# jackroos/VL-BERT

Hardware: AMD Instinct MI355X
Metric: samples/sec VL-BERT-base pretrain (seq 64+36 regions) at 1/2/4/8 MI355X (higher is better)
Workload: dtype bf16; 1 GPU; VL-BERT-base 12-layer pretrain step (fwd+bwd+clip+AdamW), 64 text + 36 regions, precomputed 2048-d region features, dropout on; global_batch=256, per_gpu_batch=256, per_gpu_caption_samples=256, per_gpu_text_only_samples=0, module=ResNetVLBERTForPretraining, seq_len=101, parallelism=dp1, hipgraph=False, arch=gfx950:sramecc+:xnack-, cus=256, forced_exchange=False, ranks=1

## Files before the change

vl-bert_amd/csrc/embed.hip:

```cpp
#include "vlb_common.h"

#define EMB_MAX_IT 8

enum { KIND_PAD = 0, KIND_TEXT = 1, KIND_OBJ = 2, KIND_END = 3 };

__global__ void seq_layout_kernel(const uint8_t* __restrict__ text_mask, const uint8_t* __restrict__ obj_mask, int B, int T, int R,
                                  int S, int32_t* __restrict__ code, int32_t* __restrict__ text_len, int32_t* __restrict__ nobj,
                                  int32_t* __restrict__ text_rows, int32_t* __restrict__ obj_rows, float* __restrict__ attn_mask) {
  const int b = blockIdx.x;
  if (threadIdx.x != 0) return;
  int n = 0;
  for (int t = 0; t < T; ++t)
    if (text_mask[b * T + t]) code[b * S + n++] = (KIND_TEXT << 16) | t;
  const int tl = n;
  for (int r = 0; r < R; ++r) {
    if (obj_mask[b * R + r]) {
      obj_rows[b * R + r] = b * S + n;
      code[b * S + n++] = (KIND_OBJ << 16) | r;
    } else {
      obj_rows[b * R + r] = -1;
    }
  }
  const int no = n - tl;
  code[b * S + n++] = (KIND_END << 16);
  for (int s = n; s < S; ++s) code[b * S + s] = (KIND_PAD << 16);
  for (int s = 0; s < S; ++s) attn_mask[b * S + s] = (s < n) ? 1.f : 0.f;
  for (int t = 0; t < T; ++t) text_rows[b * T + t] = b * S + t;
  text_len[b] = tl;
  nobj[b] = no;
}

__global__ __launch_bounds__(256) void obj_prep_fwd_kernel(const float* __restrict__ boxes, long ldbox, const float* __restrict__ im_info, long ldinfo,
                                                           const int64_t* __restrict__ mvrc_ops, const float* __restrict__ mask_emb,
                                                           bf16_t* __restrict__ out, int B, int R, uint32_t drop_thr, float drop_scale,
                                                           const uint32_t* __restrict__ seedp, uint32_t tag) {
  const int row = blockIdx.x;
  const int b = row / R;
  const float* bx = boxes + (long)row * ldbox;
  bf16_t* o = out + (long)row * 4096;
  const int tid = threadIdx.x;
  const uint32_t seed = (drop_thr && seedp) ? *seedp : 0u;
  if (!(bx[0] > -1.5f)) {
    *(uint4*)(o + tid * 8) = make_uint4(0, 0, 0, 0);
    *(uint4*)(o + 2048 + tid * 8) = make_uint4(0, 0, 0, 0);
    return;
  }
  const float W = im_info[b * ldinfo + 0], Hh = im_info[b * ldinfo + 1];
  const float x1 = bx[0], y1 = bx[1], x2 = bx[2], y2 = bx[3];
  float pos[4];
  pos[0] = (x1 + x2) / 2 / W * 100;
  pos[1] = (y1 + y2) / 2 / Hh * 100;
  pos[2] = (x2 - x1) / W * 100;
  pos[3] = (y2 - y1) / Hh * 100;
  const bool masked = mvrc_ops && mvrc_ops[row] == 1;
  const float* feat = masked ? mask_emb : (bx + 4);
#pragma unroll
  for (int part = 0; part < 2; ++part) {
    const int e0 = part * 1024 + tid * 4;
    float cv[4], fv[4];
    {
      const int which = e0 >> 9, j0 = e0 & 511;
      const bool is_cos = j0 >= 256;
#pragma unroll
      for (int k = 0; k < 4; ++k) {
        const float dim = powf(1000.0f, (float)((j0 & 255) + k) / 256.0f);
        const float a = pos[which] / dim;
        cv[k] = is_cos ? cosf(a) : sinf(a);
      }
      const float4 f = *(const float4*)(feat + e0);
      fv[0] = f.x; fv[1] = f.y; fv[2] = f.z; fv[3] = f.w;
    }
    if (drop_thr) {
      const uint32_t ic = (uint32_t)row * 4096u + (uint32_t)e0, ifeat = ic + 2048u;
      const uint32_t h0 = vlb_rng_pair(seed, tag, ic >> 1), h1 = vlb_rng_pair(seed, tag, (ic >> 1) + 1);
      const uint32_t g0 = vlb_rng_pair(seed, tag, ifeat >> 1), g1 = vlb_rng_pair(seed, tag, (ifeat >> 1) + 1);
      cv[0] = ((h0 & 0xffffu) >= drop_thr) ? cv[0] * drop_scale : 0.f;
      cv[1] = ((h0 >> 16) >= drop_thr) ? cv[1] * drop_scale : 0.f;
      cv[2] = ((h1 & 0xffffu) >= drop_thr) ? cv[2] * drop_scale : 0.f;
      cv[3] = ((h1 >> 16) >= drop_thr) ? cv[3] * drop_scale : 0.f;
      fv[0] = ((g0 & 0xffffu) >= drop_thr) ? fv[0] * drop_scale : 0.f;
      fv[1] = ((g0 >> 16) >= drop_thr) ? fv[1] * drop_scale : 0.f;
      fv[2] = ((g1 & 0xffffu) >= drop_thr) ? fv[2] * drop_scale : 0.f;
      fv[3] = ((g1 >> 16) >= drop_thr) ? fv[3] * drop_scale : 0.f;
    }
    *(uint2*)(o + e0) = make_uint2(pack2bf(cv[0], cv[1]), pack2bf(cv[2], cv[3]));
    *(uint2*)(o + 2048 + e0) = make_uint2(pack2bf(fv[0], fv[1]), pack2bf(fv[2], fv[3]));
  }
}

__global__ __launch_bounds__(256) void zero_padded_rows_kernel(bf16_t* __restrict__ x, long ld, const float* __restrict__ boxes, long ldbox,
                                                               int rows, int H) {
  const int row = blockIdx.x * 4 + (threadIdx.x >> 6), lane = threadIdx.x & 63;
  if (row >= rows || boxes[(long)row * ldbox] > -1.5f) return;
  for (int c = lane * 8; c < H; c += 512) *(uint4*)(x + (long)row * ld + c) = make_uint4(0, 0, 0, 0);
}

extern "C" int vlb_zero_padded_rows_bf16(void* x, long ld, const float* boxes, long ldbox, int rows, int H, hipStream_t stream) {
  if (rows <= 0) return VLB_OK;
  VLB_CHECK_ARG(x && boxes && H > 0 && (H % 8) == 0 && (ld % 8) == 0, "vlb_zero_padded_rows_bf16: bad argument");
  hipLaunchKernelGGL(zero_padded_rows_kernel, dim3(vlb_cdiv(rows, 4)), dim3(256), 0, stream, (bf16_t*)x, ld, boxes, ldbox, rows, H);
  VLB_CHECK_LAUNCH("vlb_zero_padded_rows_bf16");
  return VLB_OK;
}

__global__ __launch_bounds__(256) void masked_colsum_kernel(const bf16_t* __restrict__ src, long lds, const int64_t* __restrict__ sel,
                                                            int rows, int C, float* __restrict__ dst, uint32_t drop_thr,
                                                            float drop_scale, const uint32_t* __restrict__ seedp, uint32_t tag,
                                                            uint32_t row_elems, uint32_t col_off) {
  const int c = blockIdx.x * 256 + threadIdx.x;
  if (c >= C) return;
  const uint32_t seed = (drop_thr && seedp) ? *seedp : 0u;
  float s = 0.f;
  for (int r = blockIdx.y; r < rows; r += gridDim.y) {
    if (sel[r] != 1) continue;
    float v = bf2f(src[(long)r * lds + c]);
    if (drop_thr) v = vlb_keep(seed, tag, (uint32_t)r * row_elems + col_off + (uint32_t)c, drop_thr) ? v * drop_scale : 0.f;
    s += v;
  }
  atomicAdd(dst + c, s);
}

struct EmbedParams {
  const int32_t* code;
  const int32_t* text_len;
  const int64_t* text_ids;
  const int64_t* text_type;
  const bf16_t* word_emb;
  const bf16_t* pos_emb;
  const bf16_t* type_emb;
  const bf16_t* end_emb;
  const bf16_t* text_vis; long tv_sb, tv_st;
  const bf16_t* obj_vis; long ov_sb, ov_sr;
  const bf16_t* obj_ling; long ol_sb, ol_sr;
  const int64_t* obj_ling_idx;
  const float* gamma; const float* beta;
  bf16_t* pre;
  float* stats;
  bf16_t* out;
  int B, T, R, S, H, V, P;
  float eps;
  uint32_t drop_thr; float drop_scale; const uint32_t* seed; uint32_t tag;
};
// ... 391 lines not shown
  VLB_CHECK_LAUNCH("vlb_seq_layout");
  return VLB_OK;
}

extern "C" int vlb_obj_prep_fwd(const float* boxes, long ldbox, const float* im_info, long ldinfo, const int64_t* mvrc_ops,
                                const float* mask_emb, void* out, int B, int R, float drop_p, const uint32_t* seed, uint32_t tag,
                                hipStream_t stream) {
  if (B * R <= 0) return VLB_OK;
  VLB_CHECK_ARG(ldbox >= 4 + 2048 && (ldbox % 4) == 0, "vlb_obj_prep_fwd: ldbox=%ld must be >= 2052 and a multiple of 4", ldbox);
  VLB_CHECK_ARG(boxes && im_info && out && ldinfo >= 2, "vlb_obj_prep_fwd: null argument or im_info rows narrower than (width, height): ldinfo=%ld",
                ldinfo);
  VLB_CHECK_ARG(!(drop_p > 0.f) || seed, "vlb_obj_prep_fwd: dropout needs a device seed pointer");
  const uint32_t thr = vlb_drop_thr(drop_p);
  hipLaunchKernelGGL(obj_prep_fwd_kernel, dim3(B * R), dim3(256), 0, stream, boxes, ldbox, im_info, ldinfo, mvrc_ops, mask_emb, (bf16_t*)out,
                     B, R, thr, vlb_drop_scale(thr), seed, tag);
  VLB_CHECK_LAUNCH("vlb_obj_prep_fwd");
  return VLB_OK;
}

extern "C" int vlb_masked_colsum(const void* src, long lds_, const int64_t* sel, int rows, int C, float* dst, float drop_p,
                                 const uint32_t* seed, uint32_t tag, uint32_t row_elems, uint32_t col_off, hipStream_t stream) {
  if (rows <= 0 || C <= 0) return VLB_OK;
  const uint32_t thr = vlb_drop_thr(drop_p);
  int gy = rows < 64 ? rows : 64;
  hipLaunchKernelGGL(masked_colsum_kernel, dim3(vlb_cdiv(C, 256), gy), dim3(256), 0, stream, (const bf16_t*)src, lds_, sel, rows, C,
                     dst, thr, vlb_drop_scale(thr), seed, tag, row_elems, col_off);
  VLB_CHECK_LAUNCH("vlb_masked_colsum");
  return VLB_OK;
}

extern "C" int vlb_embed_fwd(const int32_t* code, const int32_t* text_len, const int64_t* text_ids, const int64_t* text_type,
                             const void* word_emb, const void* pos_emb, const void* type_emb, const void* end_emb,
                             const void* text_vis, long tv_sb, long tv_st, const void* obj_vis, long ov_sb, long ov_sr,
                             const void* obj_ling, long ol_sb, long ol_sr, const int64_t* obj_ling_idx, const float* gamma,
                             const float* beta, void* pre, float* stats, void* out, int B, int T, int R, int S, int H, int V,
                             int P, float eps, float drop_p, const uint32_t* seed, uint32_t tag, hipStream_t stream) {
  VLB_CHECK_ARG(H > 0 && (H % 4) == 0 && H <= 256 * EMB_MAX_IT, "vlb_embed_fwd: unsupported H=%d", H);
  VLB_CHECK_ARG(code && text_len && text_ids && word_emb && pos_emb && type_emb && end_emb && text_vis && obj_vis && obj_ling,
                "vlb_embed_fwd: null input");
  VLB_CHECK_ARG(!(drop_p > 0.f) || seed, "vlb_embed_fwd: dropout needs a device seed pointer");
  EmbedParams p;
  p.code = code; p.text_len = text_len; p.text_ids = text_ids; p.text_type = text_type;
  p.word_emb = (const bf16_t*)word_emb; p.pos_emb = (const bf16_t*)pos_emb; p.type_emb = (const bf16_t*)type_emb;
  p.end_emb = (const bf16_t*)end_emb;
  p.text_vis = (const bf16_t*)text_vis; p.tv_sb = tv_sb; p.tv_st = tv_st;
  p.obj_vis = (const bf16_t*)obj_vis; p.ov_sb = ov_sb; p.ov_sr = ov_sr;
  p.obj_ling = (const bf16_t*)obj_ling; p.ol_sb = ol_sb; p.ol_sr = ol_sr; p.obj_ling_idx = obj_ling_idx;
  p.gamma = gamma; p.beta = beta; p.pre = (bf16_t*)pre; p.stats = stats; p.out = (bf16_t*)out;
  p.B = B; p.T = T; p.R = R; p.S = S; p.H = H; p.V = V; p.P = P; p.eps = eps;
// ... 109 lines not shown
```

vl-bert_amd/csrc/layernorm.hip:

```cpp
#include <stdlib.h>

#include "options.h"
#include "vlb_common.h"

#define LN_MAX_IT 8
#define LN_MAX_BLOCKS 1024

__device__ unsigned int g_vlb_ln_nonfinite = 0u;

template <int NIT>
struct Row4 {
  float v[NIT][4];
};

template <int NIT>
struct Raw4 {
  uint2 w[NIT];
};

template <int NIT>
__device__ __forceinline__ void raw_load_row(const bf16_t* x, int H, int lane, Raw4<NIT>& q) {
#pragma unroll
  for (int i = 0; i < NIT; ++i) q.w[i] = *(const uint2*)(x + min((lane + 64 * i) * 4, H - 4));
}
// ... 382 lines not shown
  for (int i = 0; i < NIT; ++i)
#pragma unroll
    for (int k = 0; k < 4; ++k) {
      mine[(i * 4 + k) * 64 + lane] = gsum[i][k];
      mine[LW + (i * 4 + k) * 64 + lane] = bsum[i][k];
    }
  __syncthreads();
  for (int q = threadIdx.x; q < 2 * LW; q += 256) {
    const float v = (red[q] + red[2 * LW + q]) + (red[4 * LW + q] + red[6 * LW + q]);
    if (ws) ws[(long)blockIdx.x * 2 * LW + q] = v;
    else red[q] = v;
  }
  if (ws) return;
  __syncthreads();
  for (int c = threadIdx.x; c < 2 * H; c += 256) {
    const int which = c >= H, col = c - which * H, chunk = col >> 2;
    const float v = red[which * LW + (((chunk >> 6) * 4 + (col & 3)) << 6) + (chunk & 63)];
    float* dst = which ? dbeta : dgamma;
    if (dst) atomicAdd(dst + col, v);
  }
}


__global__ __launch_bounds__(256) void ln_param_finalize_kernel(const float* __restrict__ ws, int nslab, int LW, float* __restrict__ dgamma,
                                                                float* __restrict__ dbeta, int H, int cpl_log2) {
  __shared__ float part[4][64];
  const int tx = threadIdx.x & 63, ty = threadIdx.x >> 6;
  const int q = blockIdx.x * 64 + tx;
  float s = 0.f;
  for (int r = blockIdx.y * 4 + ty; r < nslab; r += 4 * gridDim.y) s += ws[(long)r * 2 * LW + q];
  part[ty][tx] = s;
  __syncthreads();
  if (ty == 0) {
    s = (part[0][tx] + part[1][tx]) + (part[2][tx] + part[3][tx]);
    const int r = q % LW, cpl = 1 << cpl_log2;
    const int col = ((r & 63) + 64 * (r >> (6 + cpl_log2))) * cpl + ((r >> 6) & (cpl - 1));
    if (col < H) {
      if (q < LW) { if (dgamma) atomicAdd(dgamma + col, s); }
      else if (dbeta) atomicAdd(dbeta + col, s);
    }
  }
}


extern "C" int vlb_layernorm_fwd(const void* x, long ldx, const float* gamma, const float* beta, void* y, long ldy,
                                 float* stats, int rows, int H, float eps, int x_f16, hipStream_t stream) {
  if (rows <= 0) return VLB_OK;
  VLB_CHECK_ARG(H > 0 && (H % 4) == 0 && H <= 256 * LN_MAX_IT, "vlb_layernorm_fwd: unsupported H=%d", H);
  VLB_CHECK_ARG((ldx % 4) == 0 && (ldy % 4) == 0, "vlb_layernorm_fwd: row strides must be multiples of 4");
  const int rpw_opt = vlb_opt(VLB_OPT_LN_FWD_ROWS);
  const int rpw = (rpw_opt == 1 || rpw_opt == 2 || rpw_opt == 4) ? rpw_opt : (rows >= 2 * 256 * 32 ? 2 : 1);
#define LN_FWD_R(NIT, RPW)                                                                                                              \
  hipLaunchKernelGGL((layernorm_fwd_kernel<NIT, RPW>), dim3(vlb_cdiv(rows, 4 * RPW)), dim3(256), 0, stream, (const bf16_t*)x, ldx, gamma, \
// ... 111 lines not shown
                     workspace, rows, H, x_f16, false, stream);
}

extern "C" int vlb_layernorm_bwd_slabs(int rows) {
  if (rows <= 0) return 0;
  const int blocks = ln_bwd_blocks(rows);
  return blocks > 32 ? blocks : 0;
}

struct LnFinalizeBatch {
  const float* ws[32];
  float* dgamma[32];
  float* dbeta[32];
  int nslab[32];
};

__global__ __launch_bounds__(256) void ln_param_finalize_batch_kernel(const LnFinalizeBatch b, int LW, int H, int cpl_log2) {
  __shared__ float part[4][64];
  const int e = blockIdx.z;
  const float* ws = b.ws[e];
  const int nslab = b.nslab[e];
  const int tx = threadIdx.x & 63, ty = threadIdx.x >> 6;
  const int q = blockIdx.x * 64 + tx;
  float s = 0.f;
  for (int r = blockIdx.y * 4 + ty; r < nslab; r += 4 * gridDim.y) s += ws[(long)r * 2 * LW + q];
  part[ty][tx] = s;
  __syncthreads();
  if (ty == 0) {
    s = (part[0][tx] + part[1][tx]) + (part[2][tx] + part[3][tx]);
    const int r = q % LW, cpl = 1 << cpl_log2;
    const int col = ((r & 63) + 64 * (r >> (6 + cpl_log2))) * cpl + ((r >> 6) & (cpl - 1));
    if (col < H) {
      if (q < LW) { if (b.dgamma[e]) atomicAdd(b.dgamma[e] + col, s); }
      else if (b.dbeta[e]) atomicAdd(b.dbeta[e] + col, s);
    }
  }
}

extern "C" int vlb_ln_param_finalize_batch(int n, const float* const* ws, const int* nslab, float* const* dgamma, float* const* dbeta,
                                           int H, hipStream_t stream) {
  if (n <= 0) return VLB_OK;
  VLB_CHECK_ARG(n <= 32 && ws && nslab && dgamma && dbeta, "vlb_ln_param_finalize_batch: 1..32 entries");
  VLB_CHECK_ARG(H > 0 && (H % 8) == 0 && H <= 2048, "vlb_ln_param_finalize_batch: unsupported H=%d", H);
  LnFinalizeBatch b;
  for (int i = 0; i < n; ++i) {
    VLB_CHECK_ARG(ws[i] && nslab[i] > 0, "vlb_ln_param_finalize_batch: entry %d has no partial vectors", i);
    b.ws[i] = ws[i]; b.nslab[i] = nslab[i]; b.dgamma[i] = dgamma[i]; b.dbeta[i] = dbeta[i];
  }
// ... 14 lines not shown
```

vl-bert_amd/csrc/loss.hip:

```cpp
#include "vlb_common.h"

__device__ __forceinline__ void online_merge(float& m, float& s, float m2, float s2) {
  const float mn = fmaxf(m, m2);
  if (mn == -INFINITY) return;
  s = s * __expf(m - mn) + s2 * __expf(m2 - mn);
  m = mn;
}

__device__ __forceinline__ void block_online_reduce(float& m, float& s, float* sh) {
#pragma unroll
  for (int o = 32; o > 0; o >>= 1) {
    const float m2 = __shfl_xor(m, o, 64), s2 = __shfl_xor(s, o, 64);
    online_merge(m, s, m2, s2);
  }
  const int wave = threadIdx.x >> 6, lane = threadIdx.x & 63;
  __syncthreads();
  if (lane == 0) {
    sh[wave * 2] = m;
    sh[wave * 2 + 1] = s;
  }
  __syncthreads();
  m = sh[0];
  s = sh[1];
#pragma unroll
// ... 54 lines not shown
  block_online_reduce(m, s, sh);
  const float lse = m + __logf(s);
  const float nv = fmaxf(*n_valid, 1.f);
  if (threadIdx.x == 0) atomicAdd(loss_out, (lse - bf2f(x[label])) / nv);
  const float sc = gscale / nv;
  __syncthreads();
  for (int c = threadIdx.x * 8; c < ldv; c += 2048) {
    const uint4 w = *(const uint4*)(x + c);
    const uint32_t ww[4] = {w.x, w.y, w.z, w.w};
    uint32_t o[4];
#pragma unroll
    for (int k = 0; k < 4; ++k) {
      const int c0 = c + 2 * k, c1 = c0 + 1;
      float g0 = (c0 < V) ? __expf(bflo(ww[k]) - lse) : 0.f;
      float g1 = (c1 < V) ? __expf(bfhi(ww[k]) - lse) : 0.f;
      if (c0 == label) g0 -= 1.f;
      if (c1 == label) g1 -= 1.f;
      o[k] = pack2bf(g0 * sc, g1 * sc);
    }
    *(uint4*)(x + c) = make_uint4(o[0], o[1], o[2], o[3]);
  }
}

__global__ __launch_bounds__(1024) void mlm_compact_kernel(const int64_t* __restrict__ labels, const int32_t* __restrict__ src_rows, int n,
                                                           int n_split, int V, int cap, int32_t* __restrict__ sel_pos,
                                                           int32_t* __restrict__ sel_src, int64_t* __restrict__ labels_c,
                                                           float* __restrict__ count0, float* __restrict__ count1,
                                                           int32_t* __restrict__ overflow) {
  __shared__ int wsum[16];
  __shared__ int total_s, n0_s;
  const int tid = threadIdx.x, lane = tid & 63, wave = tid >> 6;
  const int per = (n + 1023) / 1024, lo = tid * per, hi = min(n, lo + per);
  int c = 0, c0 = 0;
  for (int i = lo; i < hi; ++i) {
    const bool lab = labels[i] >= 0 && labels[i] < V;
    c += lab;
    c0 += lab && i < n_split;
  }
  int incl = c;
#pragma unroll
  for (int o = 1; o < 64; o <<= 1) {
    const int t = __shfl_up(incl, o, 64);
    if (lane >= o) incl += t;
  }
  if (lane == 63) wsum[wave] = incl;
  const float f0 = wave_sum((float)c0);
  __syncthreads();
  if (tid == 0) {
    int run = 0;
    for (int w = 0; w < 16; ++w) { const int t = wsum[w]; wsum[w] = run; run += t; }
    total_s = run;
    n0_s = 0;
  }
  __syncthreads();
  if (lane == 0 && f0 != 0.f) atomicAdd(&n0_s, (int)f0);
  __syncthreads();
  int k = wsum[wave] + incl - c;
  for (int i = lo; i < hi; ++i) {
    const long lb = labels[i];
    if (lb >= 0 && lb < V) {
      if (k < cap) {
        sel_pos[k] = i;
        sel_src[k] = src_rows[i];
        labels_c[k] = lb;
      }
      ++k;
    }
  }
  const int total = total_s;
  for (int q = total + tid; q < cap; q += 1024) {
    sel_pos[q] = -1;
    sel_src[q] = -1;
    labels_c[q] = -1;
  }
  if (tid == 0) {
    const int kept = min(total, cap), n0 = min(n0_s, kept);
    *count0 = (float)n0;
    *count1 = (float)(kept - n0);
    if (total > cap) *overflow = 1;
  }
}

extern "C" int vlb_mlm_compact(const int64_t* labels, const int32_t* src_rows, int n, int n_split, int V, int cap, int32_t* sel_pos,
                               int32_t* sel_src, int64_t* labels_c, float* count0, float* count1, int32_t* overflow, hipStream_t stream) {
  VLB_CHECK_ARG(labels && src_rows && sel_pos && sel_src && labels_c && count0 && count1 && overflow, "vlb_mlm_compact: null argument");
  VLB_CHECK_ARG(n > 0 && cap > 0 && n_split >= 0 && n_split <= n, "vlb_mlm_compact: bad sizes");
  hipLaunchKernelGGL(mlm_compact_kernel, dim3(1), dim3(1024), 0, stream, labels, src_rows, n, n_split, V, cap, sel_pos, sel_src, labels_c,
                     count0, count1, overflow);
  VLB_CHECK_LAUNCH("vlb_mlm_compact");
  return VLB_OK;
}

extern "C" int vlb_ce_fwd_bwd_compact(void* logits, long ld, int rows, int V, const int64_t* labels_c, const float* count0,
                                      const float* count1, float gscale, float* loss_out0, float* loss_out1, hipStream_t stream) {
  if (rows <= 0) return VLB_OK;
  VLB_CHECK_ARG(logits && labels_c && count0 && count1 && loss_out0 && loss_out1, "vlb_ce_fwd_bwd_compact: null argument");
  VLB_CHECK_ARG(ld >= V && (ld % 8) == 0, "vlb_ce_fwd_bwd_compact: ld=%ld must be >= V=%d and a multiple of 8", ld, V);
  hipLaunchKernelGGL(ce_fwd_bwd_kernel, dim3(rows), dim3(256), 0, stream, (bf16_t*)logits, ld, V, labels_c, count0, gscale, loss_out0,
                     (bf16_t*)nullptr, 0L, count1, loss_out1);
  VLB_CHECK_LAUNCH("vlb_ce_fwd_bwd_compact");
  return VLB_OK;
}

__global__ __launch_bounds__(256) void soft_valid_kernel(const float* __restrict__ target, long ldt, int C, int rows, float* __restrict__ tsum,
                                                         float* __restrict__ counts) {
  const int row = blockIdx.x * 4 + (threadIdx.x >> 6), lane = threadIdx.x & 63;
  if (row >= rows) return;
  const float* t = target + (long)row * ldt;
  float s = 0.f;
  for (int c = lane; c < C; c += 64) s += t[c];
  s = wave_sum(s);
  if (lane == 0) {
    tsum[row] = s;
    if (fabsf(s - 1.f) < 0.1f) atomicAdd(counts, 1.f);
  }
}

__global__ __launch_bounds__(256) void soft_ce_fwd_bwd_kernel(bf16_t* __restrict__ logits, long ld, int C, const float* __restrict__ target,
                                                              long ldt, const float* __restrict__ tsum, const float* __restrict__ n_valid,
                                                              float gscale, float* __restrict__ loss_out, bf16_t* __restrict__ logits_copy,
                                                              long ldcopy) {
  __shared__ float sh[16];
  const int row = blockIdx.x;
  bf16_t* x = logits + (long)row * ld;
  const float* t = target + (long)row * ldt;
  const int ldv = (int)ld;
  if (logits_copy) {
    bf16_t* cp = logits_copy + (long)row * ldcopy;
    for (int c = threadIdx.x; c < C; c += 256) cp[c] = x[c];
  }
  const float ts = tsum[row];
  if (!(fabsf(ts - 1.f) < 0.1f)) {
    for (int c = threadIdx.x; c < ldv; c += 256) x[c] = 0;
// ... 109 lines not shown
```

vl-bert_amd/engine.py:

```python
import math
import os
from collections import OrderedDict
from dataclasses import dataclass
from types import SimpleNamespace

import torch

from . import ops
from .side_streams import SideStreams

F32 = torch.float32
VIS_DIM = 2048
TAG_EMBED, TAG_DOWNSAMPLE = 1000, 1001


def _ru(x, m):
    return (x + m - 1) // m * m


@dataclass
class ModelConfig:
    hidden_size: int = 768
    num_hidden_layers: int = 12
    num_attention_heads: int = 12
# ... 276 lines not shown
        self.d_mlm_h, self.d_mlm_g, self.d_mlm_u = zb(BT, H), zb(BT, H), zb(BT, H)
        self.d_text_out, self.d_obj_out = zb(BT, H), zb(BR, H)
        self.d_mvrc_u = zb(BR, H)
        self.d_textvis, self.d_objvis = zf(Bt, H), zf(BR, H)
        self.d_obj_reps = zf(BR, H)
        self.d_yds = zb(BR, H)
        self.d_afeat = zb(BR, VIS_DIM)
        if core:
            self.in_text_type = torch.zeros((Bt, T), dtype=torch.int64, device=d)
            self.tv_in, self.ovl_in = zb(BT, H), zb(BR, 2 * H)
            self.tv_n, self.st_tv = zb(BT, H), zf(BT, 2)
            self.d_tv_n, self.d_ol = zf(BT, H), zf(BR, H)
            self.d_tv_in, self.d_ovl_in = zb(BT, H), zb(BR, 2 * H)
        need = [ops.wgrad_workspace_floats(n, k, rp) for n, k, rp in
                ((3 * H, H, self.Mp), (H, H, self.Mp), (I, H, self.Mp), (H, I, self.Mp), (V, H, self.BTp), (H, H, self.BTp),
                 (C, H, self.BRp), (H, H, self.BRp), (H, 2 * VIS_DIM, self.BRp))]
        need_dec = ops.wgrad_workspace_floats(self.BT, H, self.Vp)
        need.append(need_dec)
        need.append(3 * (3 * H * H + H * H + 2 * I * H) + 64)
        self.wg_ws = zf(max(max(need), 4))
        self.side = torch.cuda.Stream(device=d) if (d.type == "cuda" and os.environ.get("VLB_WGRAD_STREAM", "1") != "0") else None
        self.wg_ws_main = zf(max(need_dec, 4)) if self.side is not None else self.wg_ws
        self._hazards = SideStreams()
        self.ln_ws = zf(ops.ln_bwd_workspace_floats(H))
        n_slices = min(2 * L + 1, 32) if os.environ.get("VLB_LN_DEFER", "1") != "0" else 0
        self._ln_slices = list(zf(n_slices, ops.ln_bwd_workspace_floats(H)).unbind(0)) if n_slices else []
        self._ln_pending = []
        self.graph = None
        self._weights_dirty = True
        self.buckets = None
        self._wT_stale = self._gather_pending = self._vision_stale = False
        self._dp_hook = None
        from .parallel import force_exchange
        if (world > 1 or force_exchange()) and self._own_flat:
            from .parallel import GradBuckets
            vstart = min((o for n, o in self.P.offsets.items() if n.startswith("image_feature_extractor.") and
                          not n.startswith("image_feature_extractor.obj_downsample")), default=None)
            self.buckets = GradBuckets(self.P.grad, self.P.offsets, self.P.numel, L, group=process_group, vision_start=vstart,
                                       wire_dtype=dp_wire, mode=dp_mode)
            if self.buckets.sharded:
                self.shard_tbl = ops.ShardRanges(self.buckets.owned_rows(), d)
                self.wshard = torch.zeros(self.P.numel // world, dtype=ops.BF16, device=d)
                self.buckets.set_replicated_fp32(self._fp32_read_ranges())
        self.enc32 = None
        if encoder_fp32:
            if self.buckets is not None and self.buckets.sharded:
# ... 286 lines not shown
        else:
            self.mlm_logits.copy_(self.mlm_logits_copy)
            self.mvrc_logits.copy_(self.mvrc_logits_copy)
            losses, mcopy, vcopy = torch.zeros_like(self.losses), None, None
        nw = B * T
        if self._mlm_compact_now:
            ops.ce_fwd_bwd_compact(self.mlm_logits[:self.mlm_cap], V, self.labels_c, self.counts[0:1], self.counts[2:3], losses[0:1],
                                   losses[2:3], gscale=gscale)
        else:
            ops.ce_fwd_bwd(self.mlm_logits[:nw], V, self.in_mlm_labels.view(-1)[:nw], self.counts[0:1], losses[0:1], gscale=gscale,
                           logits_copy=mcopy[:nw] if mcopy is not None else None)
            if Ba:
                ops.ce_fwd_bwd(self.mlm_logits[nw:], V, self.in_mlm_labels.view(-1)[nw:], self.counts[2:3], losses[2:3],
                               gscale=gscale, logits_copy=mcopy[nw:] if mcopy is not None else None)
        ops.soft_ce_fwd_bwd(self.mvrc_logits, C, self.in_mvrc_labels.view(self.BR, C), self.mvrc_tsum, self.counts[1:2],
                            losses[1:2], gscale=gscale, logits_copy=vcopy)
        if self.cfg.with_rel_loss:
            if not keep:
                self.rel_logits.copy_(self.rel_logits_copy)
            ops.ce_fwd_bwd(self.rel_logits, 2, self.in_rel_label, self.counts[3:4], losses[3:4], gscale=gscale,
                           logits_copy=self.rel_logits_copy if keep else None)

    def _on_side(self, launch, items):
        self._hazards.run(self.side, launch, [dy for dy, _, _, _ in items])

    def _wgrad(self, dy, x, gw, gb):
        acc = not self._fresh_grads
        self._on_side(lambda: ops.wgrad_tn(dy, x, gw, colsum=gb, workspace=self.wg_ws, accumulate=acc), [(dy, x, gw, gb)])

    def _padded(self, items):
        pad = self._row_padded
        return [(pad.get(dy.data_ptr(), dy), pad.get(x.data_ptr(), x), gw, gb) for dy, x, gw, gb in items]

    def _wgrad_group(self, items):
        acc = not self._fresh_grads
        items = self._padded(items)
        if len({t.shape[0] for it in items for t in it[:2]}) != 1:
            items = [(dy[:self.M], x[:self.M], gw, gb) for dy, x, gw, gb in items]
        self._on_side(lambda: ops.wgrad_tn_group(items, workspace=self.wg_ws, accumulate=acc), items)

    def _wgrad_pair(self, items):
        acc = not self._fresh_grads
        items = self._padded(items)
        key = (acc,) + tuple(t.data_ptr() for it in items for t in it)
        tab = self._pair_tables.get(key)
        if tab is None:
            if self.dev.type == "cuda" and torch.cuda.is_current_stream_capturing():
# ... 115 lines not shown
            self._before_write(dQKV)
            ops.attention_bwd(self.QKV[l], mask, self.CTX[l], self.LSE[l], self.dCTX, dQKV, Bt, S, H, nh, drop_p=p_a,
                              seed=seed, tag=l * 8 + 0)
            ops.gemm_nt(dQKV, r.qkv.wT, dx_next, res=self.dZ)
            wg = [(dD2, self.G[l], r.f2.gw, r.f2.gb), (dU, self.Y1[l], r.f1.gw, r.f1.gb), (dD1, self.CTX[l], r.ao.gw, r.ao.gb),
                  (dQKV, self.X[l], r.qkv.gw, r.qkv.gb)]
            dx = dx_next
            if self._pairs and (l & 1):
                held = (l, wg)
                continue
            finished = [l]
            if held is not None:
                if not self._wgrad_pair(held[1] + wg):
                    self._wgrad_group(held[1])
                    self._wgrad_group(wg)
                finished = [held[0], l]
                held = None
            else:
                self._wgrad_group(wg)
            for lf in finished:
                if on_layer_done and (will_launch is None or will_launch(lf)):
                    self._join_side()
                    on_layer_done(lf)
        self._join_side()
        if self.core:
            self._front_core_bwd(dx, p_h)
        else:
            self._front_pretrain_bwd(dx, p_h, p_ds, on_layer_done)
        self._join_side()
        self._flush_ln()
        self._fresh_grads = False
        if on_layer_done:
            on_layer_done("embed")
            on_layer_done("vision")

    def _front_core_bwd(self, dx, p_h):
        cfg, T, R, S, Bt = self.cfg, self.T, self.R, self.S, self.Bt
        H = cfg.hidden_size
        w32, g32, seed = self.w32, self.g32, self.seed
        self.d_tv_n.zero_()
        self.d_objvis.zero_()
        self.d_ol.zero_()
        pe = "vlbert.embedding_LayerNorm."
        ops.embed_bwd(dx, self.emb_pre, self.st_emb, w32[pe + "weight"], self.lay, self.in_text, self.in_text_type, None,
                      g32["vlbert.word_embeddings.weight"], g32["vlbert.position_embeddings.weight"],
                      g32["vlbert.token_type_embeddings.weight"], g32["vlbert.end_embedding.weight"], g32[pe + "weight"],
                      g32[pe + "bias"], self.d_tv_n, (T * H, H), self.d_objvis, (R * H, H), self.d_ol, (R * H, H), Bt, T, R, S, H,
                      drop_p=p_h, seed=seed, tag=TAG_EMBED)
        ops.layernorm_bwd(self.d_tv_n, self.tv_in, self.st_tv, w32["vlbert.visual_ln_text.weight"], dx=self.d_tv_in,
                          dgamma=g32["vlbert.visual_ln_text.weight"], dbeta=g32["vlbert.visual_ln_text.bias"], workspace=self.ln_ws)
        ops.layernorm_bwd(self.d_objvis, self.ovl_in[:, :H], self.st_objvis, w32["vlbert.visual_ln_object.weight"],
                          dx=self.d_ovl_in[:, :H], dgamma=g32["vlbert.visual_ln_object.weight"],
                          dbeta=g32["vlbert.visual_ln_object.bias"], workspace=self.ln_ws)
        self.d_ovl_in[:, H:].copy_(self.d_ol)

    def _front_pretrain_bwd(self, dx, p_h, p_ds, on_layer_done=None):
        cfg, B, T, R, S, Bt, Ba = self.cfg, self.B, self.T, self.R, self.S, self.Bt, self.Ba
# ... 354 lines not shown
```

vl-bert_amd/side_streams.py:

```python
import torch


class SideStreams:
    def __init__(self):
        self._pending = {}

    def run(self, stream, fn, reads=()):
        if stream is None:
            fn()
            return
        ready = torch.cuda.Event()
        ready.record()
        with torch.cuda.stream(stream):
            stream.wait_event(ready)
            fn()
            done = torch.cuda.Event()
            done.record()
        for t in reads:
            self._pending.setdefault(t.data_ptr(), {})[stream] = done

    def before_write(self, *bufs):
        for t in bufs:
            evs = self._pending.pop(t.data_ptr(), None) if t is not None else None
            for ev in (evs or {}).values():
                torch.cuda.current_stream().wait_event(ev)

    def join(self, streams):
        for s in streams:
            ev = torch.cuda.Event()
            ev.record(s)
            torch.cuda.current_stream().wait_event(ev)
        self._pending.clear()
```

Measured before the change: 13560 samples/s.

## Parallelize embedding prep kernels and relax side-stream join before front backward

Several small kernels are reworked to be more parallel. The sequence layout and MLM compaction now use wave ballots and popcount instead of serial loops. The object positional embedding precomputes frequencies in shared memory and computes sin and cos together, and the masked column sum uses vectorized 8-wide loads with a per-block reduction. The LN finalize and row-sum loops are unrolled 8-way for memory-level parallelism. On the Python side, the full side-stream join before the front (embedding) backward is replaced by waits only on events that wrote the front-parameter gradients, letting wgrad work overlap with the embedding backward. This adds write-event tracking, which risks missing a hazard if another buffer is shared.

```diff
diff --git a/vl-bert_amd/csrc/embed.hip b/vl-bert_amd/csrc/embed.hip
--- a/vl-bert_amd/csrc/embed.hip
+++ b/vl-bert_amd/csrc/embed.hip
@@ -4,30 +4,42 @@
 
 enum { KIND_PAD = 0, KIND_TEXT = 1, KIND_OBJ = 2, KIND_END = 3 };
 
-__global__ void seq_layout_kernel(const uint8_t* __restrict__ text_mask, const uint8_t* __restrict__ obj_mask, int B, int T, int R,
-                                  int S, int32_t* __restrict__ code, int32_t* __restrict__ text_len, int32_t* __restrict__ nobj,
-                                  int32_t* __restrict__ text_rows, int32_t* __restrict__ obj_rows, float* __restrict__ attn_mask) {
-  const int b = blockIdx.x;
-  if (threadIdx.x != 0) return;
+__global__ __launch_bounds__(64) void seq_layout_kernel(const uint8_t* __restrict__ text_mask, const uint8_t* __restrict__ obj_mask, int B, int T,
+                                                        int R, int S, int32_t* __restrict__ code, int32_t* __restrict__ text_len,
+                                                        int32_t* __restrict__ nobj, int32_t* __restrict__ text_rows,
+                                                        int32_t* __restrict__ obj_rows, float* __restrict__ attn_mask) {
+  const int b = blockIdx.x, lane = threadIdx.x;
+  const unsigned long long below = (1ull << lane) - 1ull;
   int n = 0;
-  for (int t = 0; t < T; ++t)
-    if (text_mask[b * T + t]) code[b * S + n++] = (KIND_TEXT << 16) | t;
+  for (int t0 = 0; t0 < T; t0 += 64) {
+    const int t = t0 + lane;
+    const bool m = t < T && text_mask[b * T + t] != 0;
+    const unsigned long long bal = __ballot(m);
+    if (m) code[b * S + n + __popcll(bal & below)] = (KIND_TEXT << 16) | t;
+    n += __popcll(bal);
+  }
   const int tl = n;
-  for (int r = 0; r < R; ++r) {
-    if (obj_mask[b * R + r]) {
-      obj_rows[b * R + r] = b * S + n;
-      code[b * S + n++] = (KIND_OBJ << 16) | r;
-    } else {
-      obj_rows[b * R + r] = -1;
-    }
+  for (int r0 = 0; r0 < R; r0 += 64) {
+    const int r = r0 + lane;
+    const bool m = r < R && obj_mask[b * R + r] != 0;
+    const unsigned long long bal = __ballot(m);
+    const int s = n + __popcll(bal & below);
+    if (m) code[b * S + s] = (KIND_OBJ << 16) | r;
+    if (r < R) obj_rows[b * R + r] = m ? b * S + s : -1;
+    n += __popcll(bal);
   }
   const int no = n - tl;
-  code[b * S + n++] = (KIND_END << 16);
-  for (int s = n; s < S; ++s) code[b * S + s] = (KIND_PAD << 16);
-  for (int s = 0; s < S; ++s) attn_mask[b * S + s] = (s < n) ? 1.f : 0.f;
-  for (int t = 0; t < T; ++t) text_rows[b * T + t] = b * S + t;
-  text_len[b] = tl;
-  nobj[b] = no;
+  if (lane == 0) code[b * S + n] = (KIND_END << 16);
+  ++n;
+  for (int s = lane; s < S; s += 64) {
+    if (s >= n) code[b * S + s] = (KIND_PAD << 16);
+    attn_mask[b * S + s] = (s < n) ? 1.f : 0.f;
+  }
+  for (int t = lane; t < T; t += 64) text_rows[b * T + t] = b * S + t;
+  if (lane == 0) {
+    text_len[b] = tl;
+    nobj[b] = no;
+  }
 }
 
 __global__ __launch_bounds__(256) void obj_prep_fwd_kernel(const float* __restrict__ boxes, long ldbox, const float* __restrict__ im_info, long ldinfo,
@@ -45,47 +57,61 @@
     *(uint4*)(o + 2048 + tid * 8) = make_uint4(0, 0, 0, 0);
     return;
   }
+  __shared__ __attribute__((aligned(16))) float freq[256];
+  freq[tid] = powf(1000.0f, (float)tid / 256.0f);
   const float W = im_info[b * ldinfo + 0], Hh = im_info[b * ldinfo + 1];
   const float x1 = bx[0], y1 = bx[1], x2 = bx[2], y2 = bx[3];
-  float pos[4];
-  pos[0] = (x1 + x2) / 2 / W * 100;
-  pos[1] = (y1 + y2) / 2 / Hh * 100;
-  pos[2] = (x2 - x1) / W * 100;
-  pos[3] = (y2 - y1) / Hh * 100;
+  const float pos0 = (x1 + x2) / 2 / W * 100;
+  const float pos1 = (y1 + y2) / 2 / Hh * 100;
+  const float pos2 = (x2 - x1) / W * 100;
+  const float pos3 = (y2 - y1) / Hh * 100;
   const bool masked = mvrc_ops && mvrc_ops[row] == 1;
   const float* feat = masked ? mask_emb : (bx + 4);
-#pragma unroll
-  for (int part = 0; part < 2; ++part) {
-    const int e0 = part * 1024 + tid * 4;
-    float cv[4], fv[4];
-    {
-      const int which = e0 >> 9, j0 = e0 & 511;
-      const bool is_cos = j0 >= 256;
-#pragma unroll
-      for (int k = 0; k < 4; ++k) {
-        const float dim = powf(1000.0f, (float)((j0 & 255) + k) / 256.0f);
-        const float a = pos[which] / dim;
-        cv[k] = is_cos ? cosf(a) : sinf(a);
-      }
-      const float4 f = *(const float4*)(feat + e0);
-      fv[0] = f.x; fv[1] = f.y; fv[2] = f.z; fv[3] = f.w;
-    }
+  {
+    const int e0 = tid * 8;
+    const float4 f0 = *(const float4*)(feat + e0), f1 = *(const float4*)(feat + e0 + 4);
+    float fv[8] = {f0.x, f0.y, f0.z, f0.w, f1.x, f1.y, f1.z, f1.w};
     if (drop_thr) {
-      const uint32_t ic = (uint32_t)row * 4096u + (uint32_t)e0, ifeat = ic + 2048u;
-      const uint32_t h0 = vlb_rng_pair(seed, tag, ic >> 1), h1 = vlb_rng_pair(seed, tag, (ic >> 1) + 1);
-      const uint32_t g0 = vlb_rng_pair(seed, tag, ifeat >> 1), g1 = vlb_rng_pair(seed, tag, (ifeat >> 1) + 1);
-      cv[0] = ((h0 & 0xffffu) >= drop_thr) ? cv[0] * drop_scale : 0.f;
-      cv[1] = ((h0 >> 16) >= drop_thr) ? cv[1] * drop_scale : 0.f;
-      cv[2] = ((h1 & 0xffffu) >= drop_thr) ? cv[2] * drop_scale : 0.f;
-      cv[3] = ((h1 >> 16) >= drop_thr) ? cv[3] * drop_scale : 0.f;
-      fv[0] = ((g0 & 0xffffu) >= drop_thr) ? fv[0] * drop_scale : 0.f;
-      fv[1] = ((g0 >> 16) >= drop_thr) ? fv[1] * drop_scale : 0.f;
-      fv[2] = ((g1 & 0xffffu) >= drop_thr) ? fv[2] * drop_scale : 0.f;
-      fv[3] = ((g1 >> 16) >= drop_thr) ? fv[3] * drop_scale : 0.f;
-    }
-    *(uint2*)(o + e0) = make_uint2(pack2bf(cv[0], cv[1]), pack2bf(cv[2], cv[3]));
-    *(uint2*)(o + 2048 + e0) = make_uint2(pack2bf(fv[0], fv[1]), pack2bf(fv[2], fv[3]));
-  }
+      const uint32_t ifeat = (uint32_t)row * 4096u + 2048u + (uint32_t)e0;
+#pragma unroll
+      for (int q = 0; q < 4; ++q) {
+        const uint32_t g = vlb_rng_pair(seed, tag, (ifeat >> 1) + q);
+        fv[2 * q] = ((g & 0xffffu) >= drop_thr) ? fv[2 * q] * drop_scale : 0.f;
+        fv[2 * q + 1] = ((g >> 16) >= drop_thr) ? fv[2 * q + 1] * drop_scale : 0.f;
+      }
+    }
+    *(uint4*)(o + 2048 + e0) = make_uint4(pack2bf(fv[0], fv[1]), pack2bf(fv[2], fv[3]), pack2bf(fv[4], fv[5]), pack2bf(fv[6], fv[7]));
+  }
+  __syncthreads();
+  const int which = tid >> 6, j0 = (tid & 63) * 4;
+  const float p = which == 0 ? pos0 : (which == 1 ? pos1 : (which == 2 ? pos2 : pos3));
+  const float4 d4 = *(const float4*)(freq + j0);
+  const float dim[4] = {d4.x, d4.y, d4.z, d4.w};
+  float sv[4], cv[4];
+#pragma unroll
+  for (int k = 0; k < 4; ++k) {
+    const float a = p / dim[k];
+    sv[k] = sinf(a);
+    cv[k] = cosf(a);
+  }
+  if (drop_thr) {
+    const uint32_t is = (uint32_t)row * 4096u + (uint32_t)(which * 512 + j0), ic = is + 256u;
+    const uint32_t h0 = vlb_rng_pair(seed, tag, is >> 1), h1 = vlb_rng_pair(seed, tag, (is >> 1) + 1);
+    const uint32_t g0 = vlb_rng_pair(seed, tag, ic >> 1), g1 = vlb_rng_pair(seed, tag, (ic >> 1) + 1);
+    sv[0] = ((h0 & 0xffffu) >= drop_thr) ? sv[0] * drop_scale : 0.f;
+    sv[1] = ((h0 >> 16) >= drop_thr) ? sv[1] * drop_scale : 0.f;
+    sv[2] = ((h1 & 0xffffu) >= drop_thr) ? sv[2] * drop_scale : 0.f;
+    sv[3] = ((h1 >> 16) >= drop_thr) ? sv[3] * drop_scale : 0.f;
+    cv[0] = ((g0 & 0xffffu) >= drop_thr) ? cv[0] * drop_scale : 0.f;
+    cv[1] = ((g0 >> 16) >= drop_thr) ? cv[1] * drop_scale : 0.f;
+    cv[2] = ((g1 & 0xffffu) >= drop_thr) ? cv[2] * drop_scale : 0.f;
+    cv[3] = ((g1 >> 16) >= drop_thr) ? cv[3] * drop_scale : 0.f;
+  }
+  const uint32_t s01 = pack2bf(sv[0], sv[1]), s23 = pack2bf(sv[2], sv[3]), c01 = pack2bf(cv[0], cv[1]), c23 = pack2bf(cv[2], cv[3]);
+  const bool odd = tid & 1;
+  const uint32_t got0 = __shfl_xor(odd ? s01 : c01, 1, 64), got1 = __shfl_xor(odd ? s23 : c23, 1, 64);
+  const int e = which * 512 + (j0 & ~7) + (odd ? 256 : 0);
+  *(uint4*)(o + e) = odd ? make_uint4(got0, got1, c01, c23) : make_uint4(s01, s23, got0, got1);
 }
 
 __global__ __launch_bounds__(256) void zero_padded_rows_kernel(bf16_t* __restrict__ x, long ld, const float* __restrict__ boxes, long ldbox,
@@ -103,21 +129,67 @@
   return VLB_OK;
 }
 
+template <int VEC>
 __global__ __launch_bounds__(256) void masked_colsum_kernel(const bf16_t* __restrict__ src, long lds, const int64_t* __restrict__ sel,
                                                             int rows, int C, float* __restrict__ dst, uint32_t drop_thr,
                                                             float drop_scale, const uint32_t* __restrict__ seedp, uint32_t tag,
                                                             uint32_t row_elems, uint32_t col_off) {
-  const int c = blockIdx.x * 256 + threadIdx.x;
-  if (c >= C) return;
+  __shared__ float part[4][64 * VEC];
+  const int lane = threadIdx.x & 63, wave = threadIdx.x >> 6;
+  const int c0 = (blockIdx.x * 64 + lane) * VEC;
+  const bool live = c0 < C;
   const uint32_t seed = (drop_thr && seedp) ? *seedp : 0u;
-  float s = 0.f;
-  for (int r = blockIdx.y; r < rows; r += gridDim.y) {
-    if (sel[r] != 1) continue;
-    float v = bf2f(src[(long)r * lds + c]);
-    if (drop_thr) v = vlb_keep(seed, tag, (uint32_t)r * row_elems + col_off + (uint32_t)c, drop_thr) ? v * drop_scale : 0.f;
-    s += v;
-  }
-  atomicAdd(dst + c, s);
+  float s[VEC];
+#pragma unroll
+  for (int k = 0; k < VEC; ++k) s[k] = 0.f;
+  for (int base = (blockIdx.y * 4 + wave) * 64; base < rows; base += 4 * gridDim.y * 64) {
+    const int rl = base + lane;
+    unsigned long long m = __ballot(rl < rows && sel[rl] == 1);
+    while (m) {
+      int r[4];
+      bool ok[4];
+#pragma unroll
+      for (int u = 0; u < 4; ++u) {
+        ok[u] = m != 0;
+        r[u] = base + (ok[u] ? __builtin_ctzll(m) : 0);
+        m &= m - 1;
+      }
+      [[maybe_unused]] uint4 w[4];
+      [[maybe_unused]] bf16_t w1[4];
+#pragma unroll
+      for (int u = 0; u < 4; ++u) {
+        if (ok[u] && live) {
+          if constexpr (VEC == 8) w[u] = *(const uint4*)(src + (long)r[u] * lds + c0);
+          else w1[u] = src[(long)r[u] * lds + c0];
+        }
+      }
+#pragma unroll
+      for (int u = 0; u < 4; ++u) {
+        if (ok[u] && live) {
+          float v[VEC];
+          if constexpr (VEC == 8) {
+            v[0] = bflo(w[u].x); v[1] = bfhi(w[u].x); v[2] = bflo(w[u].y); v[3] = bfhi(w[u].y);
+            v[4] = bflo(w[u].z); v[5] = bfhi(w[u].z); v[6] = bflo(w[u].w); v[7] = bfhi(w[u].w);
+          } else {
+            v[0] = bf2f(w1[u]);
+          }
+#pragma unroll
+          for (int k = 0; k < VEC; ++k) {
+            if (drop_thr)
+              v[k] = vlb_keep(seed, tag, (uint32_t)r[u] * row_elems + col_off + (uint32_t)(c0 + k), drop_thr) ? v[k] * drop_scale : 0.f;
+            s[k] += v[k];
+          }
+        }
+      }
+    }
+  }
+#pragma unroll
+  for (int k = 0; k < VEC; ++k) part[wave][lane * VEC + k] = s[k];
+  __syncthreads();
+  for (int i = threadIdx.x; i < 64 * VEC; i += 256) {
+    const int c = blockIdx.x * 64 * VEC + i;
+    if (c < C) atomicAdd(dst + c, (part[0][i] + part[1][i]) + (part[2][i] + part[3][i]));
+  }
 }
 
 struct EmbedParams {
@@ -555,9 +627,13 @@
                                  const uint32_t* seed, uint32_t tag, uint32_t row_elems, uint32_t col_off, hipStream_t stream) {
   if (rows <= 0 || C <= 0) return VLB_OK;
   const uint32_t thr = vlb_drop_thr(drop_p);
-  int gy = rows < 64 ? rows : 64;
-  hipLaunchKernelGGL(masked_colsum_kernel, dim3(vlb_cdiv(C, 256), gy), dim3(256), 0, stream, (const bf16_t*)src, lds_, sel, rows, C,
-                     dst, thr, vlb_drop_scale(thr), seed, tag, row_elems, col_off);
+  const int chunks4 = vlb_cdiv(vlb_cdiv(rows, 64), 4), gy = chunks4 < 64 ? chunks4 : 64;
+  if ((C % 8) == 0 && (lds_ % 8) == 0 && ((uintptr_t)src % 16) == 0)
+    hipLaunchKernelGGL(masked_colsum_kernel<8>, dim3(vlb_cdiv(C, 512), gy), dim3(256), 0, stream, (const bf16_t*)src, lds_, sel, rows, C,
+                       dst, thr, vlb_drop_scale(thr), seed, tag, row_elems, col_off);
+  else
+    hipLaunchKernelGGL(masked_colsum_kernel<1>, dim3(vlb_cdiv(C, 64), gy), dim3(256), 0, stream, (const bf16_t*)src, lds_, sel, rows, C,
+                       dst, thr, vlb_drop_scale(thr), seed, tag, row_elems, col_off);
   VLB_CHECK_LAUNCH("vlb_masked_colsum");
   return VLB_OK;
 }
diff --git a/vl-bert_amd/csrc/layernorm.hip b/vl-bert_amd/csrc/layernorm.hip
--- a/vl-bert_amd/csrc/layernorm.hip
+++ b/vl-bert_amd/csrc/layernorm.hip
@@ -428,13 +428,25 @@
 }
 
 
+__device__ __forceinline__ float ln_slab_colsum(const float* __restrict__ ws, int nslab, int LW, int q, int r0, int step) {
+  float s = 0.f;
+  for (int r = r0; r < nslab; r += 8 * step) {
+    float v[8];
+#pragma unroll
+    for (int u = 0; u < 8; ++u) v[u] = (r + u * step < nslab) ? ws[(long)(r + u * step) * 2 * LW + q] : 0.f;
+#pragma unroll
+    for (int u = 0; u < 8; ++u)
+      if (r + u * step < nslab) s += v[u];
+  }
+  return s;
+}
+
 __global__ __launch_bounds__(256) void ln_param_finalize_kernel(const float* __restrict__ ws, int nslab, int LW, float* __restrict__ dgamma,
                                                                 float* __restrict__ dbeta, int H, int cpl_log2) {
   __shared__ float part[4][64];
   const int tx = threadIdx.x & 63, ty = threadIdx.x >> 6;
   const int q = blockIdx.x * 64 + tx;
-  float s = 0.f;
-  for (int r = blockIdx.y * 4 + ty; r < nslab; r += 4 * gridDim.y) s += ws[(long)r * 2 * LW + q];
+  float s = ln_slab_colsum(ws, nslab, LW, q, blockIdx.y * 4 + ty, 4 * gridDim.y);
   part[ty][tx] = s;
   __syncthreads();
   if (ty == 0) {
@@ -592,8 +604,7 @@
   const int nslab = b.nslab[e];
   const int tx = threadIdx.x & 63, ty = threadIdx.x >> 6;
   const int q = blockIdx.x * 64 + tx;
-  float s = 0.f;
-  for (int r = blockIdx.y * 4 + ty; r < nslab; r += 4 * gridDim.y) s += ws[(long)r * 2 * LW + q];
+  float s = ln_slab_colsum(ws, nslab, LW, q, blockIdx.y * 4 + ty, 4 * gridDim.y);
   part[ty][tx] = s;
   __syncthreads();
   if (ty == 0) {
diff --git a/vl-bert_amd/csrc/loss.hip b/vl-bert_amd/csrc/loss.hip
--- a/vl-bert_amd/csrc/loss.hip
+++ b/vl-bert_amd/csrc/loss.hip
@@ -100,59 +100,69 @@
   }
 }
 
+#define MLM_TILE_CHUNKS 16
 __global__ __launch_bounds__(1024) void mlm_compact_kernel(const int64_t* __restrict__ labels, const int32_t* __restrict__ src_rows, int n,
                                                            int n_split, int V, int cap, int32_t* __restrict__ sel_pos,
                                                            int32_t* __restrict__ sel_src, int64_t* __restrict__ labels_c,
                                                            float* __restrict__ count0, float* __restrict__ count1,
                                                            int32_t* __restrict__ overflow) {
-  __shared__ int wsum[16];
-  __shared__ int total_s, n0_s;
+  __shared__ int wsum[16], wsum0[16];
   const int tid = threadIdx.x, lane = tid & 63, wave = tid >> 6;
-  const int per = (n + 1023) / 1024, lo = tid * per, hi = min(n, lo + per);
-  int c = 0, c0 = 0;
-  for (int i = lo; i < hi; ++i) {
-    const bool lab = labels[i] >= 0 && labels[i] < V;
-    c += lab;
-    c0 += lab && i < n_split;
-  }
-  int incl = c;
-#pragma unroll
-  for (int o = 1; o < 64; o <<= 1) {
-    const int t = __shfl_up(incl, o, 64);
-    if (lane >= o) incl += t;
-  }
-  if (lane == 63) wsum[wave] = incl;
-  const float f0 = wave_sum((float)c0);
-  __syncthreads();
-  if (tid == 0) {
-    int run = 0;
-    for (int w = 0; w < 16; ++w) { const int t = wsum[w]; wsum[w] = run; run += t; }
-    total_s = run;
-    n0_s = 0;
-  }
-  __syncthreads();
-  if (lane == 0 && f0 != 0.f) atomicAdd(&n0_s, (int)f0);
-  __syncthreads();
-  int k = wsum[wave] + incl - c;
-  for (int i = lo; i < hi; ++i) {
-    const long lb = labels[i];
-    if (lb >= 0 && lb < V) {
-      if (k < cap) {
-        sel_pos[k] = i;
-        sel_src[k] = src_rows[i];
-        labels_c[k] = lb;
+  const unsigned long long below = (1ull << lane) - 1ull;
+  int total = 0, n0 = 0;
+  for (int tile0 = 0; tile0 < n; tile0 += 1024 * MLM_TILE_CHUNKS) {
+    const int first = tile0 + wave * MLM_TILE_CHUNKS * 64;
+    int lab[MLM_TILE_CHUNKS];
+    unsigned long long bal[MLM_TILE_CHUNKS];
+    int wtot = 0, wtot0 = 0;
+#pragma unroll
+    for (int i = 0; i < MLM_TILE_CHUNKS; ++i) {
+      const int idx = first + i * 64 + lane;
+      const int64_t l = (idx < n) ? labels[idx] : (int64_t)-1;
+      lab[i] = (int)l;
+      bal[i] = __ballot(l >= 0 && l < V);
+    }
+#pragma unroll
+    for (int i = 0; i < MLM_TILE_CHUNKS; ++i) {
+      const int d = n_split - (first + i * 64);
+      const unsigned long long front = d <= 0 ? 0ull : (d >= 64 ? ~0ull : (1ull << d) - 1ull);
+      wtot += __popcll(bal[i]);
+      wtot0 += __popcll(bal[i] & front);
+    }
+    __syncthreads();
+    if (lane == 0) {
+      wsum[wave] = wtot;
+      wsum0[wave] = wtot0;
+    }
+    __syncthreads();
+    int k = total;
+#pragma unroll
+    for (int w = 0; w < 16; ++w) {
+      if (w < wave) k += wsum[w];
+      total += wsum[w];
+      n0 += wsum0[w];
+    }
+#pragma unroll
+    for (int i = 0; i < MLM_TILE_CHUNKS; ++i) {
+      if ((bal[i] >> lane) & 1ull) {
+        const int kk = k + __popcll(bal[i] & below), idx = first + i * 64 + lane;
+        if (kk < cap) {
+          sel_pos[kk] = idx;
+          sel_src[kk] = src_rows[idx];
+          labels_c[kk] = (int64_t)lab[i];
+        }
       }
-      ++k;
-    }
-  }
-  const int total = total_s;
+      k += __popcll(bal[i]);
+    }
+  }
   for (int q = total + tid; q < cap; q += 1024) {
     sel_pos[q] = -1;
     sel_src[q] = -1;
     labels_c[q] = -1;
   }
   if (tid == 0) {
-    const int kept = min(total, cap), n0 = min(n0_s, kept);
+    const int kept = min(total, cap);
+    n0 = min(n0, kept);
     *count0 = (float)n0;
     *count1 = (float)(kept - n0);
     if (total > cap) *overflow = 1;
@@ -186,7 +196,14 @@
   if (row >= rows) return;
   const float* t = target + (long)row * ldt;
   float s = 0.f;
-  for (int c = lane; c < C; c += 64) s += t[c];
+  for (int c = lane; c < C; c += 512) {
+    float v[8];
+#pragma unroll
+    for (int u = 0; u < 8; ++u) v[u] = (c + 64 * u < C) ? t[c + 64 * u] : 0.f;
+#pragma unroll
+    for (int u = 0; u < 8; ++u)
+      if (c + 64 * u < C) s += v[u];
+  }
   s = wave_sum(s);
   if (lane == 0) {
     tsum[row] = s;
diff --git a/vl-bert_amd/engine.py b/vl-bert_amd/engine.py
--- a/vl-bert_amd/engine.py
+++ b/vl-bert_amd/engine.py
@@ -322,6 +322,7 @@
         self.side = torch.cuda.Stream(device=d) if (d.type == "cuda" and os.environ.get("VLB_WGRAD_STREAM", "1") != "0") else None
         self.wg_ws_main = zf(max(need_dec, 4)) if self.side is not None else self.wg_ws
         self._hazards = SideStreams()
+        self._front_join = os.environ.get("VLB_FRONT_JOIN", "0") != "0"
         self.ln_ws = zf(ops.ln_bwd_workspace_floats(H))
         n_slices = min(2 * L + 1, 32) if os.environ.get("VLB_LN_DEFER", "1") != "0" else 0
         self._ln_slices = list(zf(n_slices, ops.ln_bwd_workspace_floats(H)).unbind(0)) if n_slices else []
@@ -654,7 +655,7 @@
                            logits_copy=self.rel_logits_copy if keep else None)
 
     def _on_side(self, launch, items):
-        self._hazards.run(self.side, launch, [dy for dy, _, _, _ in items])
+        self._hazards.run(self.side, launch, [dy for dy, _, _, _ in items], writes=[g for _, _, gw, gb in items for g in (gw, gb)])
 
     def _wgrad(self, dy, x, gw, gb):
         acc = not self._fresh_grads
@@ -816,7 +817,10 @@
                 if on_layer_done and (will_launch is None or will_launch(lf)):
                     self._join_side()
                     on_layer_done(lf)
-        self._join_side()
+        if on_layer_done or self._front_join:
+            self._join_side()
+        else:
+            self._hazards.before_accumulate(*self._front_grads())
         if self.core:
             self._front_core_bwd(dx, p_h)
         else:
@@ -827,6 +831,16 @@
         if on_layer_done:
             on_layer_done("embed")
             on_layer_done("vision")
+
+    FRONT_GRADS = ("vlbert.word_embeddings.weight", "vlbert.position_embeddings.weight", "vlbert.token_type_embeddings.weight",
+                   "vlbert.end_embedding.weight", "vlbert.embedding_LayerNorm.weight", "vlbert.embedding_LayerNorm.bias",
+                   "vlbert.visual_ln_text.weight", "vlbert.visual_ln_text.bias", "vlbert.visual_ln_object.weight",
+                   "vlbert.visual_ln_object.bias", "object_linguistic_embeddings.weight", "object_mask_word_embedding.weight",
+                   "aux_text_visual_embedding.weight", "object_mask_visual_embedding.weight", "image_feature_extractor.obj_downsample.1.weight",
+                   "image_feature_extractor.obj_downsample.1.bias")
+
+    def _front_grads(self):
+        return [self.g32[n] for n in self.FRONT_GRADS if n in self.g32]
 
     def _front_core_bwd(self, dx, p_h):
         cfg, T, R, S, Bt = self.cfg, self.T, self.R, self.S, self.Bt
diff --git a/vl-bert_amd/side_streams.py b/vl-bert_amd/side_streams.py
--- a/vl-bert_amd/side_streams.py
+++ b/vl-bert_amd/side_streams.py
@@ -4,8 +4,9 @@
 class SideStreams:
     def __init__(self):
         self._pending = {}
+        self._written = {}
 
-    def run(self, stream, fn, reads=()):
+    def run(self, stream, fn, reads=(), writes=()):
         if stream is None:
             fn()
             return
@@ -18,6 +19,21 @@
             done.record()
         for t in reads:
             self._pending.setdefault(t.data_ptr(), {})[stream] = done
+        for t in writes:
+            if t is not None:
+                self._written.setdefault(t.data_ptr(), []).append(done)
+
+    def writers(self, *bufs):
+        evs = []
+        for t in bufs:
+            for ev in self._written.get(t.data_ptr(), ()) if t is not None else ():
+                if not any(ev is e for e in evs):
+                    evs.append(ev)
+        return evs
+
+    def before_accumulate(self, *bufs):
+        for ev in self.writers(*bufs):
+            torch.cuda.current_stream().wait_event(ev)
 
     def before_write(self, *bufs):
         for t in bufs:
@@ -31,3 +47,4 @@
             ev.record(s)
             torch.cuda.current_stream().wait_event(ev)
         self._pending.clear()
+        self._written.clear()
```

Measured after the change: 13780 samples/s, median of 6. 1.02x the previous value.
